# hammershock/3dgs-avatar-release

Hardware: AMD Instinct MI355X
Metric: render fps (fwd+bwd) @200k Gaussians 1024x1024 SH3 (higher is better)
Workload: dtype f32; 1 GPU; config3: 200k Gaussians, 1024x1024, SH deg 3, forward+backward; shs+scales+rotations inputs, L1 loss (L1 fused into the rasterizer: l1_target); tile_rect=1, l1=fused, long_lists=0, gaussians=200000, width=1024, height=1024, sh_degree=3, frames_per_rank=1857, total_frames=1857, ranks=1, backend=none, parallelism=frames sharded x1

## Files before the change

### 3dgs-avatar-release_amd/csrc/binning.hip

```cpp
#include "common.h"

__global__ __launch_bounds__(256) void first_pair_kernel(const uint32_t* __restrict__ tiles,
                                                         const uint32_t* __restrict__ wave_tiles, float* __restrict__ rec,
                                                         int P, unsigned long long* __restrict__ count,
                                                         unsigned long long* host_count) {
    __shared__ unsigned long long wb[4];
    const int tid = threadIdx.x, lane = tid & 63, wid = tid >> 6;
    const int w0 = 4 * (int)blockIdx.x;
    unsigned long long before = 0;
    for (int w = tid; w < w0; w += 256) before += wave_tiles[w];
#pragma unroll
    for (int d = 32; d >= 1; d >>= 1) before += __shfl_xor(before, d, 64);
    if (lane == 0) wb[wid] = before;
    const int i = blockIdx.x * 256 + tid;
    const uint32_t v = i < P ? tiles[i] : 0u;
    uint32_t x = v;
#pragma unroll
    for (int d = 1; d < 64; d <<= 1) {
        const uint32_t y = __shfl_up(x, d, 64);
        if (lane >= d) x += y;
    }
    __syncthreads();
    const unsigned long long block_base = (wb[0] + wb[1]) + (wb[2] + wb[3]);
    uint32_t woff = 0;
// ... 349 lines not shown
        uint32_t* __restrict__ nstash = &wmax[1];
        if (tid == 0) *nstash = 0u;
        __syncthreads();
        const uint32_t nx = (uint32_t)__popc(xmask);
        for (int pos = tid; pos < ntiles; pos += 1024) {
            const uint32_t ov = order[pos];
            if (!(ov >> 31)) continue;
            const int t = (int)(ov & 0x7FFFFFFFu);
            const uint32_t nch = (tile_work(ranges, keys, mode, t) + ch - 1u) / ch;
            const uint32_t u0 = atomicAdd(&wmax[0], nch);
            const uint32_t ph = (uint32_t)pos % (2u * nx);
            uint32_t pick = ph < nx ? ph : 2u * nx - 1u - ph, best = 0;
            for (uint32_t x = 0; x < 8; x++) {
                if ((xmask >> x) & 1u) {
                    if (pick == 0u) { best = x; break; }
                    pick--;
                }
            }
            const uint32_t i0 = atomicAdd(&wsum[8 + best], 4u * nch);
            const uint32_t k = atomicAdd(nstash, 1u);
            stash[4 * k] = (uint32_t)t;
            stash[4 * k + 1] = u0;
            stash[4 * k + 2] = i0 | (best << 28);
            stash[4 * k + 3] = nch;
        }
        __syncthreads();
        const uint32_t nk = *nstash;
        for (uint32_t k = (uint32_t)wid; k < nk; k += 16) {
            const uint32_t t = stash[4 * k], u0 = stash[4 * k + 1], ib = stash[4 * k + 2], nch = stash[4 * k + 3];
            uint32_t* __restrict__ items = ll.cw_items + (size_t)(ib >> 28) * (FWDC_MAX_UNITS * 4) + (ib & 0x0FFFFFFFu);
            for (uint32_t c = (uint32_t)lane; c < nch; c += 64) ll.cw_units[u0 + c] = make_uint2(t, c | (nch << 16));
            for (uint32_t i = (uint32_t)lane; i < 4u * nch; i += 64) items[i] = (u0 + (i >> 2)) * 4u + (i & 3u);
        }
    }
    if (ll.cw_hdr) {
        __syncthreads();
        if (tid == 0) {
            ll.cw_hdr[0] = (mode == 2 && ch) ? wmax[0] : 0u;
            ll.cw_hdr[1] = ch;
        }
        if (tid < 8) ll.cw_hdr[4 + tid] = (mode == 2 && ch) ? wsum[8 + tid] : 0u;
    }
}

template <bool HELD>
__global__ __launch_bounds__(1024) void tile_order_kernel(const uint2* __restrict__ ranges,
                                                          const uint32_t* __restrict__ keys, int mode, int ntiles,
                                                          uint32_t* __restrict__ order, const PairCount pc,
                                                          const FillJob fill, const LongLists ll) {
    if (blockIdx.x > 0) {
        if (fill.clean && *fill.clean == MARKS_CLEAN) return;
        const uint4 ones = make_uint4(0xFFFFFFFFu, 0xFFFFFFFFu, 0xFFFFFFFFu, 0xFFFFFFFFu);
        for (size_t k = (size_t)(blockIdx.x - 1) * 1024 + threadIdx.x; k < fill.quads; k += (size_t)(gridDim.x - 1) * 1024)
            if (fill.stream) store_stream(&fill.ptr[k], ones); else fill.ptr[k] = ones;
        return;
    }
    __shared__ uint32_t hist[1024];
    __shared__ uint32_t wmax[16];
    __shared__ uint32_t wsum[16];
    if (mode < 0) return;
    tile_order_body<HELD>(ranges, keys, mode, ntiles, order, pc, ll, hist, wmax, wsum);
}

#define BM_LD 33
#ifndef TW_STOP_AFTER
#define TW_STOP_AFTER 99
#endif
template <bool CW>
__global__ __launch_bounds__(TBK_THREADS) void tile_write_kernel(const uint4* __restrict__ ranklist,
                                                                 const uint32_t* __restrict__ seg_start, int P, int gx,
                                                                 int gy, int nbx, int nblocks, int nseg, int ntiles,
                                                                 const uint32_t* __restrict__ seg_cnt,
                                                                 const uint32_t* __restrict__ tile_tot,
                                                                 uint2* __restrict__ ranges, uint32_t* __restrict__ order,
                                                                 uint32_t* __restrict__ point_list, const PairCount pc,
                                                                 const LongLists ll) {
    __shared__ uint32_t m_id[TBK_BUF];
    __shared__ unsigned short m_rc[TBK_BUF];
    __shared__ uint32_t bitmap[TB_TILES * BM_LD];
    __shared__ uint32_t dst[TB_TILES];
    __shared__ uint32_t wcnt[TBK_WAVES];
    __shared__ unsigned long long sb_scratch[20];
    static_assert(TBK_THREADS == 1024 && TBK_WAVES == 16 && TB_H <= 4 && TB_TILES * BM_LD >= 1024 && TB_TILES >= 32, "the ordering job borrows bitmap / dst");
    if (blockIdx.x == 0) {
        if (CW) {
            if (ntiles <= 32 * 1024) tile_order_body<true>(nullptr, tile_tot, 2, ntiles, order, pc, ll, bitmap, dst, dst + 16);
            else tile_order_body<false>(nullptr, tile_tot, 2, ntiles, order, pc, ll, bitmap, dst, dst + 16);
        } else if (ntiles <= 32 * 1024) {
            tile_order_plain<true>(nullptr, tile_tot, 2, ntiles, order, pc, ll, bitmap, dst, dst + 16);
        } else {
            tile_order_plain<false>(nullptr, tile_tot, 2, ntiles, order, pc, ll, bitmap, dst, dst + 16);
        }
        return;
    }
    const int tid = threadIdx.x, lane = tid & 63, wid = tid >> 6;
    const int b = ((int)blockIdx.x - 1) % nblocks, sg = ((int)blockIdx.x - 1) / nblocks;
    const int r0 = min(P, (int)seg_start[sg] * 256), r1 = min(P, (int)seg_start[sg + 1] * 256);
    const int bx0 = (b % nbx) * TB_W, by0 = (b / nbx) * TB_H;
    const int bx1 = min(gx, bx0 + TB_W), by1 = min(gy, by0 + TB_H);
    const unsigned long long frame_pairs = *pc.dev;
    const bool fits = frame_pairs <= (unsigned long long)pc.cap;
    uint32_t my_dst = 0;
    {
        const int t_blk0 = by0 * gx + bx0;
        uint32_t part = 0;
        for (int t0 = 0; t0 < t_blk0; t0 += 4 * TBK_THREADS) {
            uint32_t v[4];
#pragma unroll
            for (int k = 0; k < 4; k++) v[k] = t0 + k * TBK_THREADS + tid < t_blk0 ? tile_tot[t0 + k * TBK_THREADS + tid] : 0u;
            part += (v[0] + v[1]) + (v[2] + v[3]);
        }
        const int ty = by0 + wid, tx = bx0 + lane;
        const bool row_ok = tid < TB_TILES && ty < by1;
        const int t_row0 = ty * gx + bx0, t = t_row0 + lane;
        const bool tile_ok = row_ok && tx < bx1;
        uint32_t tot = 0, pre = 0, rowsum = 0;
        if (row_ok) {
            for (int k = lane; k < gx; k += 64) rowsum += t_row0 + k < ntiles ? tile_tot[t_row0 + k] : 0u;
            if (tile_ok) {
                tot = tile_tot[t];
                for (int s0 = 0; s0 < sg; s0 += 8) {
                    uint32_t v[8];
#pragma unroll
                    for (int k = 0; k < 8; k++) v[k] = (s0 + k < sg) ? seg_cnt[(size_t)(s0 + k) * ntiles + t] : 0u;
#pragma unroll
                    for (int k = 0; k < 8; k++) pre += v[k];
                }
            }
        }
        part = wave_sum(part);
        rowsum = wave_sum(rowsum);
        uint32_t* s_part = reinterpret_cast<uint32_t*>(sb_scratch);
        if (lane == 0) {
            s_part[wid] = part;
            if (wid < TB_H) s_part[16 + wid] = rowsum;
        }
        __syncthreads();
        if (row_ok) {
            uint32_t before = 0;
            for (int w = 0; w < TBK_WAVES; w++) before += s_part[w];
            for (int r = 0; r < wid; r++) before += s_part[16 + r];
            const uint32_t x = wave_scan_incl(tot);
            const uint32_t first = before + x - tot;
            if (sg == 0 && tile_ok) ranges[t] = fits ? make_uint2(first, first + tot) : make_uint2(0u, 0u);
            my_dst = first + pre;
        }
        __syncthreads();
    }
    if (TW_STOP_AFTER <= 1) return;
    if (!fits || !point_list) return;
    for (int k = tid; k < TB_TILES * BM_LD; k += TBK_THREADS) bitmap[k] = 0u;
    uint4 e[TBK_LPL];
    auto load_trip = [&](const int rb) {
#pragma unroll
        for (int k = 0; k < TBK_LPL; k++) {
            const int r = rb + wid * (64 * TBK_LPL) + k * 64 + lane;
            e[k] = r < r1 ? ranklist[r] : make_uint4(0, 0, 0, 0);
        }
    };
    if (TW_STOP_AFTER <= 2) return;
    load_trip(r0);
    if (tid < TB_TILES) dst[tid] = my_dst;
    const unsigned long long lt_mask = (lane == 0) ? 0ull : (~0ull >> (64 - lane));
    int count = 0;
    const int grp = lane >> 4, gl = lane & 15;

    auto process_batch = [&](const int n) {
        const int nw = (n + 31) >> 5;
        for (int m0 = wid * 4; m0 < n; m0 += TBK_WAVES * 4) {
            const int m = m0 + grp;
            if (m < n) {
                const uint32_t rc = m_rc[m];
                const uint32_t lw = ((rc >> 8) & 63u) + 1u, lh = ((rc >> 14) & 3u) + 1u;
                const uint32_t area = lw * lh, lx = rc & 63u, ly = (rc >> 6) & 3u;
                for (uint32_t j = (uint32_t)gl; j < area; j += 16u) {
                    const uint32_t dy = (j >= lw ? 1u : 0u) + (j >= 2u * lw ? 1u : 0u) + (j >= 3u * lw ? 1u : 0u);
                    const uint32_t lt = (ly + dy) * TB_W + lx + (j - dy * lw);
                    atomicOr(&bitmap[lt * BM_LD + (m >> 5)], 1u << (m & 31));
                }
// ... 145 lines not shown
```

### 3dgs-avatar-release_amd/csrc/capi.hip

```cpp
#include "common.h"
#include "boundary.h"
#include <string.h>
#include <stdlib.h>
#include <atomic>
#include <chrono>
#include <mutex>
#include <vector>

static thread_local int g_last_hip = 0;
static thread_local const char* g_last_stage = "";
void gs_set_error(int hip_err, const char* stage) {
    g_last_hip = hip_err;
    g_last_stage = stage;
}

struct TuneSwitch {
    const char* name;
    int key, def;
    const char* env;
    bool (*ok)(int);
};
static const TuneSwitch k_tune[GS_TUNE_COUNT] = {
    {"xcd_map", GS_TUNE_XCD_MAP, 1, nullptr, nullptr},
    {"depth_sort", GS_TUNE_DEPTH_SORT, 1, nullptr, nullptr},
    {"nt_stores", GS_TUNE_NT_STORES, 1, nullptr, nullptr},
    {"bwd_chunks", GS_TUNE_BWD_CHUNKS, 1, nullptr, nullptr},
    {"fwd4", GS_TUNE_FWD4, 1, "GSPLAT_FWD4", nullptr},
    {"small_tiles", GS_TUNE_SMALL_TILES, BWD_CHUNK_MAX_TILES, nullptr, nullptr},
    {"shared_qlist", GS_TUNE_SHARED_QLIST, 1, nullptr, nullptr},
    {"ones_fast", GS_TUNE_ONES_FAST, 1, nullptr, nullptr},
    {"bwd_order", GS_TUNE_BWD_ORDER, 1, nullptr, nullptr},
    {"fwd_marks", GS_TUNE_FWD_MARKS, 1, nullptr, nullptr},
    {"fwdc_ch", GS_TUNE_FWDC_CH, (int)FWDC_CH_MIN, "GSPLAT_FWDC_CH", [](int v) { return v >= 64 && (v & (v - 1)) == 0; }},
    {"fwdc_div", GS_TUNE_FWDC_DIV, (int)FWD4_TOTAL_DIV, "GSPLAT_FWDC_DIV", [](int v) { return v >= 1; }},
};
struct TuneState {
    std::atomic<int> v[GS_TUNE_COUNT];
    TuneState() {
        for (const TuneSwitch& t : k_tune) {
            int value = t.def;
            if (const char* e = t.env ? getenv(t.env) : nullptr) {
                const int x = atoi(e);
                if (!t.ok || t.ok(x)) value = x;
            }
            v[t.key].store(value);
        }
    }
};
static TuneState& tune_state() {
    static TuneState st;
    return st;
}
int gs_tune_get(int key) {
    return (key >= 0 && key < GS_TUNE_COUNT) ? tune_state().v[key].load(std::memory_order_relaxed) : 0;
}

struct ProfRec { const char* name; hipEvent_t a, b; };
struct ProfState {
    bool on = false;
    bool armed = false;
    int nested = 0;
    char filter[32] = {0};
    std::vector<ProfRec> recs;
    std::vector<hipEvent_t> pool;
    hipEvent_t get() {
        if (!pool.empty()) { hipEvent_t e = pool.back(); pool.pop_back(); return e; }
        hipEvent_t e = nullptr;
        (void)hipEventCreate(&e);
        return e;
    }
};
static ProfState g_prof;
static std::mutex g_prof_mu;
bool profiling_on() { return g_prof.on; }
void gs_prof_begin(const char* stage, hipStream_t s) {
    if (!g_prof.on) return;
    std::lock_guard<std::mutex> lk(g_prof_mu);
    if (g_prof.armed) { g_prof.nested++; return; }
    g_prof.armed = g_prof.on && (g_prof.filter[0] == 0 || strcmp(g_prof.filter, stage) == 0);
    if (!g_prof.armed) return;
    ProfRec r{stage, g_prof.get(), g_prof.get()};
    (void)hipEventRecord(r.a, s);
    g_prof.recs.push_back(r);
}
void gs_prof_end(hipStream_t s) {
    if (!g_prof.on) return;
    std::lock_guard<std::mutex> lk(g_prof_mu);
    if (!g_prof.armed || g_prof.recs.empty()) return;
    if (g_prof.nested > 0) { g_prof.nested--; return; }
    (void)hipEventRecord(g_prof.recs.back().b, s);
    g_prof.armed = false;
}

static int validate(const GsFwdArgs* a) {
    if (!a) return GS_E_BAD_ARG;
    if (a->P < 0 || a->W <= 0 || a->H <= 0) return GS_E_BAD_ARG;
    if (!a->bg || !a->viewmatrix || !a->projmatrix || !a->campos) return GS_E_BAD_ARG;
    if (a->P > 0 && (!a->means3D || !a->opacities)) return GS_E_BAD_ARG;
    if ((a->shs != nullptr) == (a->colors_precomp != nullptr)) return GS_E_EXCLUSIVE;
    const bool sr = a->scales != nullptr && a->rotations != nullptr;
    if ((a->scales != nullptr) != (a->rotations != nullptr)) return GS_E_EXCLUSIVE;
    if (sr == (a->cov3D_precomp != nullptr)) return GS_E_EXCLUSIVE;
    if (a->shs) {
        if (a->sh_degree < 0 || a->sh_degree > 3) return GS_E_BAD_ARG;
        if (a->M < (a->sh_degree + 1) * (a->sh_degree + 1)) return GS_E_BAD_ARG;
        if (a->M > 16) return GS_E_BAD_ARG;
    }
    if (!aligned(a->rotations, 16)) return GS_E_BAD_ARG;
    if ((a->W + TILE - 1) / TILE > 0xFFFF || (a->H + TILE - 1) / TILE > 0xFFFF) return GS_E_TOO_LARGE;
    return GS_OK;
}

bool stream_is_capturing(void* stream) {
    hipStreamCaptureStatus st = hipStreamCaptureStatusNone;
    const hipError_t e = hipStreamIsCapturing((hipStream_t)stream, &st);
    if (e != hipSuccess) {
        (void)hipGetLastError();
        return e == hipErrorStreamCaptureImplicit || e == hipErrorStreamCaptureUnsupported || e == hipErrorStreamCaptureInvalidated;
    }
    return st != hipStreamCaptureStatusNone;
}

__global__ void zero_words_kernel(uint32_t* __restrict__ p, size_t words) {
    for (size_t k = (size_t)blockIdx.x * blockDim.x + threadIdx.x; k < words; k += (size_t)gridDim.x * blockDim.x) p[k] = 0u;
}
int gs_zero_async(void* ptr, size_t bytes, const char* stage, hipStream_t s) {
    const size_t words = bytes / 4;
    if (words == 0) return GS_OK;
    const size_t blocks = (words + 255) / 256;
    hipLaunchKernelGGL(zero_words_kernel, dim3((unsigned)(blocks < 1024 ? blocks : 1024)), dim3(256), 0, s, (uint32_t*)ptr, words);
    const hipError_t e = hipGetLastError();
    if (e != hipSuccess) { gs_set_error((int)e, stage); return GS_E_HIP; }
    return GS_OK;
}

__global__ __launch_bounds__(256) void clock_probe_kernel(unsigned long long* __restrict__ out, int iters, float seed, float* __restrict__ sink) {
    const unsigned long long t0 = __builtin_readcyclecounter(), r0 = __builtin_amdgcn_s_memrealtime();
    float a[8];
#pragma unroll
    for (int i = 0; i < 8; i++) a[i] = seed + (float)i + (float)threadIdx.x * 1e-3f;
    for (int it = 0; it < iters; it++) {
#pragma unroll
        for (int u = 0; u < 4; u++)
#pragma unroll
            for (int i = 0; i < 8; i++) a[i] = __builtin_fmaf(a[i], 1.0001f, 0.5f);
    }
    float sum = 0.f;
#pragma unroll
    for (int i = 0; i < 8; i++) sum += a[i];
    if (sum == 12345.678f) sink[0] = sum;
    if (threadIdx.x == 0) {
        const unsigned long long t1 = __builtin_readcyclecounter(), r1 = __builtin_amdgcn_s_memrealtime();
        atomicAdd(&out[0], t1 - t0);
        atomicAdd(&out[1], r1 - r0);
    }
}

__global__ __launch_bounds__(64) void xcc_probe_kernel(uint32_t* __restrict__ out) {
    if (threadIdx.x == 0) out[blockIdx.x] = xcc_id();
}

template <class Void, class VoidBin, class G, class B, class I, class Own>
static int frame_states(const GsFwdArgs* a, Void* geom, size_t geom_bytes, VoidBin* binning, size_t binning_bytes, Void* img,
                        size_t img_bytes, int64_t D, G* g, B* b, I* im, Own own) {
    int rc = validate(a);
    if (rc != GS_OK) return rc;
    if (!geom || !img || D < 0 || (D > 0 && !binning)) return GS_E_BAD_ARG;
    if ((rc = own()) != GS_OK) return rc;
    *g = geom_state(geom, a->P);
    *im = img_state(img, a->W, a->H, a->long_lists);
    *b = bin_state(D > 0 ? binning : nullptr, D);
    if (geom_bytes < g->total || img_bytes < im->total || (D > 0 && binning_bytes < b->total)) return GS_E_WORKSPACE;
    return GS_OK;
}

template <class T> static T* writable(T* p) { return p; }
template <class T> static T* writable(const T* p) { return const_cast<T*>(p); }
template <bool RO>
static QuadLists quad_lists(const ImgViewT<RO>& im, const BinView& b, int long_lists) {
    QuadLists ql;
    ql.qlist = b.qlist;
    ql.ncon_c = writable(im.ncon_c);
    ql.qcount = writable(im.qcount);
    ql.chunks = gs_tune_get(GS_TUNE_BWD_CHUNKS) ? im.bwd_chunks : 1;
    ql.four_waves = forward_small_image(im.ntiles, long_lists) ? 1 : 0;
    ql.ckpt = ql.chunks > 1 ? writable(im.ckpt) : nullptr;
    ql.ck_start = ql.chunks > 1 ? writable(im.ck_start) : nullptr;
    return ql;
}
template <bool RO>
static void quad_lists_chunked(QuadLists& ql, const ImgView& own, const ImgViewT<RO>& list) {
    ql.chunked = 1;
    ql.cw_hdr = list.cw_hdr;
    ql.cw_units = list.cw_units;
    ql.cw_items = list.cw_items;
    ql.cw_q = own.cw_q;
    ql.cw_flag = own.cw_flag;
    ql.cw_done = own.cw_done;
    ql.cw_rec = own.cw_rec;
}
static int sync_if_debug(const GsFwdArgs* a, const char* stage, hipStream_t s) {
    if (!a->debug) return GS_OK;
    const hipError_t e = hipStreamSynchronize(s);
// ... 390 lines not shown
        default: return GS_E_BAD_ARG;
    }
    return GS_OK;
}
int gs_image_field(void* img, int32_t W, int32_t H, int32_t field, void** out) {
    if (!img || !out) return GS_E_BAD_ARG;
    const ImgView im = img_state(img, W, H, 0);
    void* p = nullptr;
    switch (field) {
        case GS_IMG_RANGES: p = im.ranges; break;
        case GS_IMG_N_CONTRIB: p = im.n_contrib; break;
        case GS_IMG_FINAL_T: p = im.final_T; break;
        case GS_IMG_QCOUNT: p = im.qcount; break;
        case GS_IMG_NCON_C: p = im.ncon_c; break;
        case GS_IMG_ORDER: p = im.order; break;
        case GS_IMG_CW_HDR: p = im.cw_hdr; break;
        case GS_IMG_CW_UNITS: p = im.cw_units; break;
        case GS_IMG_CW_FLAG: p = im.cw_flag; break;
        case GS_IMG_CW_REC: p = im.cw_rec; break;
    }
    if (!p) return GS_E_BAD_ARG;
    *out = p;
    return GS_OK;
}

int gs_profile_enable(int on) {
    std::lock_guard<std::mutex> lk(g_prof_mu);
    g_prof.on = on != 0;
    return GS_OK;
}
int gs_profile_reserve(int n_events) {
    std::lock_guard<std::mutex> lk(g_prof_mu);
    hipEvent_t last = nullptr;
    while ((int)g_prof.pool.size() < n_events) {
        hipEvent_t e = nullptr;
        if (hipEventCreate(&e) != hipSuccess) return GS_E_HIP;
        (void)hipEventRecord(e, nullptr);
        last = e;
        g_prof.pool.push_back(e);
    }
    if (last) (void)hipEventSynchronize(last);
    return GS_OK;
}
int gs_profile_filter(const char* stage) {
    std::lock_guard<std::mutex> lk(g_prof_mu);
    memset(g_prof.filter, 0, sizeof(g_prof.filter));
    if (stage) strncpy(g_prof.filter, stage, sizeof(g_prof.filter) - 1);
    return GS_OK;
}
int gs_profile_collect(int max, const char** names, float* ms, int32_t* launches, int32_t* n_out) {
    if (max < 0 || !n_out || (max > 0 && (!names || !ms || !launches))) return GS_E_BAD_ARG;
    std::lock_guard<std::mutex> lk(g_prof_mu);
    int n = 0;
    for (auto& r : g_prof.recs) {
        float t = 0.f;
        hipError_t e = hipEventSynchronize(r.b);
        if (e == hipSuccess) e = hipEventElapsedTime(&t, r.a, r.b);
        if (e != hipSuccess) { gs_set_error((int)e, "profile.collect"); t = 0.f; }
        int k = 0;
        for (; k < n; k++) if (names[k] == r.name) break;
        if (k == n) {
            if (n < max) { names[n] = r.name; ms[n] = 0.f; launches[n] = 0; n++; } else k = -1;
        }
        if (k >= 0) { ms[k] += t; launches[k] += 1; }
        g_prof.pool.push_back(r.a);
        g_prof.pool.push_back(r.b);
    }
    g_prof.recs.clear();
    *n_out = n;
    return GS_OK;
}

int gs_tuning(const char* name, int value) {
    if (!name) return GS_E_BAD_ARG;
    for (const TuneSwitch& t : k_tune) {
        if (strcmp(name, t.name) != 0) continue;
        if (t.ok && !t.ok(value)) return GS_E_BAD_ARG;
        tune_state().v[t.key].store(value);
        return GS_OK;
    }
    return GS_E_BAD_ARG;
}

const char* gs_status_string(int code) {
    switch (code) {
        case GS_OK: return "ok";
        case GS_E_BAD_ARG: return "bad argument (null required pointer, non-positive size, unsupported SH degree / more than 16 SH coefficients, or rotations not 16-byte aligned)";
        case GS_E_EXCLUSIVE: return "provide exactly one of shs/colors_precomp and exactly one of (scales, rotations)/cov3D_precomp";
        case GS_E_TOO_LARGE: return "num_rendered or tile grid exceeds the supported index space";
        case GS_E_HIP: return "HIP error";
        case GS_E_WORKSPACE: return "state/workspace buffer smaller than gs_*_bytes requires";
        case GS_E_CAPTURE: return "the stream is being captured into a graph and this call is not capture-safe with these arguments (include/gsplat_mi355.h, \"Stream capture\"); nothing was enqueued";
        default: return "unknown status";
    }
}
int gs_last_hip_error(void) { return g_last_hip; }
const char* gs_last_stage(void) { return g_last_stage; }
const char* gs_build_info(void) { return "gsplat_mi355 gfx950 wave64 tile16 rec48"; }

}
```

### 3dgs-avatar-release_amd/csrc/common.h

```cpp
#pragma once
#include <hip/hip_runtime.h>
#include <stdint.h>
#include <stddef.h>
#include <type_traits>
#include "../../include/gsplat_mi355.h"

#define TILE 16
#define WAVE 64
#define REC_F 12
#define GS_MAX_PAIRS 0x3FFFFFFFll

static inline size_t align_up(size_t x, size_t a) { return (x + a - 1) / a * a; }

#define SORT_ITEMS 4096
#define SORT_SMALL_N (1 << 20)
#define SORT_TOTALS_REPL 16
static inline size_t sort_table_words(size_t n) {
    const size_t items = n <= (size_t)SORT_SMALL_N ? 1024 : SORT_ITEMS;
    return (size_t)256 * ((n + items - 1) / items + 4 * SORT_TOTALS_REPL);
}
#define SCAN_ITEMS 2048

#ifndef DS_ITEMS
#define DS_ITEMS 2048
// ... 9 lines not shown
#define TB_MAX_SEG 64
enum { COUNT_PAIRS = 0, COUNT_NOT_ONES = 2, COUNT_ZERO_BYTES = 24 };
struct GeomLayout {
    size_t rec, depths, tiles, clamped, key0, key1, val0, val1, ranklist, chunk_pairs, wsum, wkmin, wkmax, hist, count,
        ds_tmp, ds_tmp2, ds_cnt, ds_pre, ds_tot, ds_loc, ds_grp, ds_range, seg_start, total;
    int nblk_sort, nwaves, ds_nb, ds_blocks;
};
static inline GeomLayout geom_layout(int P) {
    GeomLayout L;
    size_t o = 0;
    size_t n = (size_t)(P > 0 ? P : 1);
    auto take = [&](size_t bytes) { size_t at = o; o = align_up(o + bytes, 256); return at; };
    L.nblk_sort = (int)((n + SORT_ITEMS - 1) / SORT_ITEMS);
    L.nwaves = (int)((n + 255) / 256) * 4;
    L.rec = take(n * REC_F * 4);
    L.depths = take(n * 4);
    L.tiles = take(n * 4);
    L.clamped = take(n * 4);
    L.key0 = take(n * 4);
    L.key1 = take(n * 4);
    L.val0 = take(n * 4);
    L.val1 = take(n * 4);
    L.ranklist = take(n * 16);
    L.chunk_pairs = take(((n + 255) / 256) * 4);
    L.wsum = take((size_t)L.nwaves * 4);
    L.wkmin = take((size_t)L.nwaves * 4);
    L.wkmax = take((size_t)L.nwaves * 4);
    L.hist = take(sort_table_words(n) * 4);
    L.count = take(64);
    L.ds_nb = ds_buckets(P);
    L.ds_blocks = (int)((n + DS_ITEMS - 1) / DS_ITEMS);
    L.ds_tmp = take(n * 8);
    L.ds_tmp2 = take(n * 8);
    L.ds_cnt = take((size_t)L.ds_blocks * (L.ds_nb + 1) * 4);
    L.ds_pre = take((size_t)L.ds_blocks * (L.ds_nb + 1) * 4);
    L.ds_tot = take((size_t)(L.ds_nb + 1) * 4);
    L.ds_loc = take((size_t)(L.ds_nb + 1) * 4);
    L.ds_grp = take((size_t)((L.ds_nb + 1 + 63) / 64) * 4);
    L.ds_range = take(16);
    L.seg_start = take((size_t)(TB_MAX_SEG + 2) * 4);
    L.total = o;
    return L;
}

struct BinLayout {
    size_t point_list, qlist, marks, marks_flag, total;
};
static inline BinLayout bin_layout(int64_t D) {
    BinLayout L;
    size_t o = 0;
    size_t n = (size_t)(D > 0 ? D : 1);
    auto take = [&](size_t bytes) { size_t at = o; o = align_up(o + bytes, 256); return at; };
    L.point_list = take(n * 4);
    L.qlist = take(n * 16);
    L.marks = take(n * 16);
    L.marks_flag = take(4);
    L.total = o;
    return L;
}

#define TB_W 64
#ifndef TB_H
#define TB_H 4
#endif
#define TB_TILES (TB_W * TB_H)
struct BinGrid { int nbx, nby, nblocks, nseg_max; };
static inline BinGrid bin_grid(int gx, int gy) {
    BinGrid G;
    G.nbx = (gx + TB_W - 1) / TB_W;
    G.nby = (gy + TB_H - 1) / TB_H;
    G.nblocks = G.nbx * G.nby;
#ifndef TB_TARGET_WGS
#define TB_TARGET_WGS 512
#endif
    int s = (TB_TARGET_WGS + G.nblocks - 1) / G.nblocks;
    G.nseg_max = s < 1 ? 1 : (s > TB_MAX_SEG ? TB_MAX_SEG : s);
    return G;
}
static inline int bin_segments(const BinGrid& G, int P) {
    int s = (P + 1023) / 1024;
    if (s < 1) s = 1;
    return s < G.nseg_max ? s : G.nseg_max;
}

enum { GS_TUNE_XCD_MAP = 0, GS_TUNE_DEPTH_SORT = 1, GS_TUNE_NT_STORES = 2, GS_TUNE_BWD_CHUNKS = 3, GS_TUNE_FWD4 = 4, GS_TUNE_SMALL_TILES = 5, GS_TUNE_SHARED_QLIST = 6, GS_TUNE_ONES_FAST = 7, GS_TUNE_BWD_ORDER = 8, GS_TUNE_FWD_MARKS = 9, GS_TUNE_FWDC_CH = 10, GS_TUNE_FWDC_DIV = 11, GS_TUNE_COUNT = 12 };
int gs_tune_get(int key);

#define BWD_CH 128
#define BWD_KMAX 16
#define BWD_CHUNK_MAX_TILES 2048
#define FWD4_MAX_TILES 2048
#define FWD4_MIN_LIST 512u
#ifndef FWD4_TOTAL_DIV
#define FWD4_TOTAL_DIV 320ull
#endif

#define FWDC_CH_MIN 256u
#define FWDC_SPARSE_PAIRS 524288ull
#define FWDC_MAX_UNITS 4096
#define FWDC_MAX_TILES (FWDC_MAX_UNITS / 2)
#define FWDC_Q_WORDS (8 * FWDC_MAX_UNITS * 4)
#define FWDC_Q_BYTES ((size_t)FWDC_Q_WORDS * 4 + 64)
#ifdef FWDC_PROF
#define FWDC_SLOTS 9
#else
#define FWDC_SLOTS 8
#endif
#define FWDC_DEAD 0x80000000u
#define FWDC_SPIN_MAX (1 << 16)
struct ImgLayout {
    size_t ranges, n_contrib, final_T, ncon_c, tile_nmax, order, seg_cnt, tile_tot, all_ones, cw_flag, cw_done, cw_q, tile_zero_bytes, l1_part, ckpt, ck_start, cw_hdr, cw_units, cw_items, cw_rec, total;
    int gx, gy, bwd_chunks;
};
static inline bool few_long_lists_mode(int ntiles, int long_lists) {
    return ntiles <= gs_tune_get(GS_TUNE_SMALL_TILES) || long_lists != 0;
}
static inline ImgLayout img_layout(int W, int H, int long_lists = 0) {
    ImgLayout L;
    size_t o = 0;
    auto take = [&](size_t bytes) { size_t at = o; o = align_up(o + bytes, 256); return at; };
    L.gx = (W + TILE - 1) / TILE;
    L.gy = (H + TILE - 1) / TILE;
    const size_t nt = (size_t)L.gx * L.gy;
    L.ranges = take(nt * 8);
    L.n_contrib = take((size_t)W * H * 4);
    L.final_T = take((size_t)W * H * 4);
    L.ncon_c = take((size_t)W * H * 4);
    L.tile_nmax = take(nt * 16);
    L.order = take(nt * 4);
    L.seg_cnt = take(nt * 4 * (size_t)bin_grid(L.gx, L.gy).nseg_max);
    L.tile_tot = take(nt * 4);
    L.all_ones = take(4);
    L.tile_zero_bytes = L.all_ones + 4 - L.tile_tot;
    const bool fl = few_long_lists_mode((int)nt, long_lists);
    const bool cw = fl && gs_tune_get(GS_TUNE_FWD4) == 2;
    L.cw_flag = L.cw_done = L.cw_q = 0;
    if (cw) {
        L.cw_flag = take((size_t)FWDC_MAX_UNITS * 4 * 4);
        L.cw_done = take(nt * 16);
        L.cw_q = take(FWDC_Q_BYTES);
        L.tile_zero_bytes = L.cw_q + FWDC_Q_BYTES - L.tile_tot;
    }
    L.l1_part = take(nt * 16);
    L.bwd_chunks = fl ? BWD_KMAX : 1;
    L.ckpt = take(nt * 4 * (size_t)(L.bwd_chunks - 1) * 64 * 16);
    L.ck_start = take(nt * 4 * (size_t)L.bwd_chunks * 4);
    L.cw_hdr = L.cw_units = L.cw_items = L.cw_rec = 0;
    if (cw) {
        L.cw_hdr = take(64);
        L.cw_units = take((size_t)FWDC_MAX_UNITS * 8);
        L.cw_items = take((size_t)FWDC_Q_WORDS * 4);
        L.cw_rec = take((size_t)FWDC_MAX_UNITS * 4 * FWDC_SLOTS * 64 * 4);
    }
    L.total = o;
    return L;
}

template <bool RO>
struct StateCarve {
    typename std::conditional<RO, const char, char>::type* base;
    StateCarve(typename std::conditional<RO, const void, void>::type* state) : base(static_cast<decltype(base)>(state)) {}
    template <class T>
    void operator()(T*& field, size_t offset, bool present = true) const {
        field = (base && present) ? reinterpret_cast<T*>(base + offset) : nullptr;
    }
};
template <bool RO>
struct GeomViewT {
    template <class T> using ptr = typename std::conditional<RO, const T, T>::type*;
// ... 403 lines not shown
```

### 3dgs-avatar-release_amd/csrc/gaussian_bwd.hip

```cpp
#include "common.h"
#include "gs_math.h"
#include "blend.h"

#ifndef GB_THREADS
#define GB_THREADS 256
#endif

__global__ __launch_bounds__(256) void segment_reduce_kernel(int P, const int32_t* __restrict__ radii,
                                                             const float4* __restrict__ rec,
                                                             const uint32_t* __restrict__ tiles,
                                                             const uint32_t* __restrict__ q8,
                                                             const float4* __restrict__ qrows,
                                                             float4* __restrict__ sums, uint32_t* __restrict__ marks_flag) {
    const int t = blockIdx.x * blockDim.x + threadIdx.x;
    if (t == 0 && marks_flag) *marks_flag = 0u;
    const int i = t >> 4, j = t & 15;
    const int rs = j >> 1, h = j & 1;
    float a0 = 0.f, a1 = 0.f, a2 = 0.f, a3 = 0.f, a8 = 0.f;
    const bool in = i < P;
    float4 r0 = make_float4(0.f, 0.f, 0.f, 0.f), r1 = r0;
    if (in && radii[i] > 0) {
        const uint32_t off = __float_as_uint(rec[(size_t)i * 3 + 2].y);
        const uint32_t nrows = 4u * tiles[i];
        if (j < 2) {
// ... 221 lines not shown
                            dx += SH_C3[0] * SHC(9) * 3.f * 2.f * xy + SH_C3[1] * SHC(10) * yz + SH_C3[2] * SHC(11) * -2.f * xy +
                                  SH_C3[3] * SHC(12) * -3.f * 2.f * xz + SH_C3[4] * SHC(13) * (-3.f * xx + 4.f * zz - yy) +
                                  SH_C3[5] * SHC(14) * 2.f * xz + SH_C3[6] * SHC(15) * 3.f * (xx - yy);
                            dy += SH_C3[0] * SHC(9) * 3.f * (xx - yy) + SH_C3[1] * SHC(10) * xz + SH_C3[2] * SHC(11) * (-3.f * yy + 4.f * zz - xx) +
                                  SH_C3[3] * SHC(12) * -3.f * 2.f * yz + SH_C3[4] * SHC(13) * -2.f * xy +
                                  SH_C3[5] * SHC(14) * -2.f * yz + SH_C3[6] * SHC(15) * -3.f * 2.f * xy;
                            dz += SH_C3[1] * SHC(10) * xy + SH_C3[2] * SHC(11) * 4.f * 2.f * yz + SH_C3[3] * SHC(12) * 3.f * (2.f * zz - xx - yy) +
                                  SH_C3[4] * SHC(13) * 4.f * 2.f * xz + SH_C3[5] * SHC(14) * (xx - yy);
                        }
                    }
                }
                for (int k = (deg + 1) * (deg + 1); k < M; k++) GSH(k) = 0.f;
#undef SHC
#undef GSH
                ddir[0] += dx * g;
                ddir[1] += dy * g;
                ddir[2] += dz * g;
            }
            const float sum2 = dox * dox + doy * doy + doz * doz;
            const float invsum32 = 1.0f / sqrtf(sum2 * sum2 * sum2);
            gm[0] += ((+sum2 - dox * dox) * ddir[0] - doy * dox * ddir[1] - doz * dox * ddir[2]) * invsum32;
            gm[1] += (-dox * doy * ddir[0] + (sum2 - doy * doy) * ddir[1] - doz * doy * ddir[2]) * invsum32;
            gm[2] += (-dox * doz * ddir[0] - doy * doz * ddir[1] + (sum2 - doz * doz) * ddir[2]) * invsum32;
        }
        if (!cov3D_precomp) {
            float R[3][3];
            quat_to_R(q, R);
            const float sv[3] = {scale_modifier * sc.x, scale_modifier * sc.y, scale_modifier * sc.z};
            const float dS[3][3] = {{gc[0], 0.5f * gc[1], 0.5f * gc[2]},
                                    {0.5f * gc[1], gc[3], 0.5f * gc[4]},
                                    {0.5f * gc[2], 0.5f * gc[4], gc[5]}};
            float L[3][3], dL[3][3], dR[3][3];
#pragma unroll
            for (int r_ = 0; r_ < 3; r_++)
#pragma unroll
                for (int c_ = 0; c_ < 3; c_++) L[r_][c_] = R[r_][c_] * sv[c_];
#pragma unroll
            for (int r_ = 0; r_ < 3; r_++)
#pragma unroll
                for (int c_ = 0; c_ < 3; c_++)
                    dL[r_][c_] = 2.0f * (dS[r_][0] * L[0][c_] + dS[r_][1] * L[1][c_] + dS[r_][2] * L[2][c_]);
#pragma unroll
            for (int c_ = 0; c_ < 3; c_++) {
                gs[c_] = R[0][c_] * dL[0][c_] + R[1][c_] * dL[1][c_] + R[2][c_] * dL[2][c_];
#pragma unroll
                for (int r_ = 0; r_ < 3; r_++) dR[r_][c_] = dL[r_][c_] * sv[c_];
            }
            const float r = q.x, x = q.y, y = q.z, z = q.w;
            gq[0] = 2 * z * (dR[1][0] - dR[0][1]) + 2 * y * (dR[0][2] - dR[2][0]) + 2 * x * (dR[2][1] - dR[1][2]);
            gq[1] = 2 * y * (dR[0][1] + dR[1][0]) + 2 * z * (dR[0][2] + dR[2][0]) + 2 * r * (dR[2][1] - dR[1][2]) - 4 * x * (dR[2][2] + dR[1][1]);
            gq[2] = 2 * x * (dR[0][1] + dR[1][0]) + 2 * r * (dR[0][2] - dR[2][0]) + 2 * z * (dR[2][1] + dR[1][2]) - 4 * y * (dR[2][2] + dR[0][0]);
            gq[3] = 2 * r * (dR[1][0] - dR[0][1]) + 2 * x * (dR[0][2] + dR[2][0]) + 2 * y * (dR[2][1] + dR[1][2]) - 4 * z * (dR[1][1] + dR[0][0]);
        }
    } else if (shs) {
        float* gsh = sh_tile + threadIdx.x * ld;
        for (int k = 0; k < M * 3; k++) gsh[k] = 0.f;
    }
    dL_dmeans3D[3 * i] = gm[0];
    dL_dmeans3D[3 * i + 1] = gm[1];
    dL_dmeans3D[3 * i + 2] = gm[2];
#pragma unroll
    for (int k = 0; k < 6; k++) dL_dcov3D[6 * i + k] = gc[k];
    if (dL_dscales) {
        dL_dscales[3 * i] = gs[0];
        dL_dscales[3 * i + 1] = gs[1];
        dL_dscales[3 * i + 2] = gs[2];
    }
    if (dL_drotations) reinterpret_cast<float4*>(dL_drotations)[i] = make_float4(gq[0], gq[1], gq[2], gq[3]);
    }
    if (shs) {
        __syncthreads();
        sh_tile_store(dL_dsh + (size_t)row0 * M * 3, sh_tile, nrows, M * 3, ld);
    }
}

int launch_gaussian_backward(const GsFwdArgs& a, const int32_t* radii, const float* rec, const uint32_t* tiles,
                             const uint32_t* clamped, const uint32_t* q8, const float* qrows, float* sums,
                             uint32_t* marks_flag, const GsGrads& g, hipStream_t s) {
    const float fy = a.H / (2.0f * a.tanfovy), fx = a.W / (2.0f * a.tanfovx);
    hipLaunchKernelGGL(segment_reduce_kernel, dim3((unsigned)(((size_t)a.P * 16 + 255) / 256)), dim3(256), 0, s, a.P, radii,
                       reinterpret_cast<const float4*>(rec), tiles, q8,
                       reinterpret_cast<const float4*>(qrows), reinterpret_cast<float4*>(sums), marks_flag);
    GS_LAUNCH_CHECK("segment_reduce", a.debug, s);
    const size_t lds = a.shs ? (size_t)GB_THREADS * ((3 * a.M) | 1) * sizeof(float) : 0;
    hipLaunchKernelGGL(a.antialiasing ? gaussian_bwd_kernel<true> : gaussian_bwd_kernel<false>,
                       dim3((a.P + GB_THREADS - 1) / GB_THREADS), dim3(GB_THREADS), lds, s, a.P, a.sh_degree, a.M, a.means3D,
                       a.scales, a.scale_modifier, a.rotations, a.shs, a.cov3D_precomp, a.viewmatrix, a.projmatrix,
                       a.campos, a.W, a.H, a.tanfovx, a.tanfovy, fx, fy, radii, clamped,
                       reinterpret_cast<const float4*>(sums), g.dL_dmeans3D, g.dL_dmeans2D,
                       g.dL_dsh, g.dL_dcolors, g.dL_dopacity, g.dL_dscales, g.dL_drotations, g.dL_dcov3D,
                       reinterpret_cast<const float4*>(rec));
    GS_LAUNCH_CHECK("gaussian_backward", a.debug, s);
    return GS_OK;
}
```

### 3dgs-avatar-release_amd/csrc/gs_math.h

```cpp
#pragma once
#include <hip/hip_runtime.h>
#include <stdint.h>

#define SH_C0 0.28209479177387814f
#define SH_C1 0.4886025119029199f
__device__ __constant__ static const float SH_C2[5] = {1.0925484305920792f, -1.0925484305920792f, 0.31539156525252005f,
                                                       -1.0925484305920792f, 0.5462742152960396f};
__device__ __constant__ static const float SH_C3[7] = {-0.5900435899266435f, 2.890611442640554f,
                                                       -0.4570457994644658f, 0.3731763325901154f,
                                                       -0.4570457994644658f, 1.445305721320277f,
                                                       -0.5900435899266435f};

__device__ __forceinline__ float3 xform4x3(const float3 p, const float* m) {
    return make_float3(m[0] * p.x + m[4] * p.y + m[8] * p.z + m[12], m[1] * p.x + m[5] * p.y + m[9] * p.z + m[13],
                       m[2] * p.x + m[6] * p.y + m[10] * p.z + m[14]);
}
__device__ __forceinline__ float4 xform4x4(const float3 p, const float* m) {
    return make_float4(m[0] * p.x + m[4] * p.y + m[8] * p.z + m[12], m[1] * p.x + m[5] * p.y + m[9] * p.z + m[13],
                       m[2] * p.x + m[6] * p.y + m[10] * p.z + m[14], m[3] * p.x + m[7] * p.y + m[11] * p.z + m[15]);
}

__device__ __forceinline__ void quat_to_R(const float4 q, float R[3][3]) {
    const float r = q.x, x = q.y, y = q.z, z = q.w;
    R[0][0] = 1.f - 2.f * (y * y + z * z);
// ... 94 lines not shown
    const float thr = 2.0f * ln_upper_bound(x) + 0.002f;
    const float cond = (cov_a * cov_c) / det;
    const float widen = 1.0f + cond * 1.9073486e-6f;
    if (!(det > 0.0f) || !(widen <= 2.0f)) {
        *hx = *hy = 1.0e7f;
        return true;
    }
    const float thr_w = thr * widen;
    *hx = fminf(sqrtf(thr_w * cov_a), 1.0e7f);
    *hy = fminf(sqrtf(thr_w * cov_c), 1.0e7f);
    return true;
}

__device__ __forceinline__ float3 sh_eval_dir(int deg, const float x, const float y, const float z,
                                              const float* __restrict__ sh, uint32_t* clamped) {
    float out[3];
    uint32_t cl = 0;
#pragma unroll
    for (int c = 0; c < 3; c++) {
#define SHC(k) sh[(k) * 3 + c]
        float r = SH_C0 * SHC(0);
        if (deg > 0) {
            r = r - SH_C1 * y * SHC(1) + SH_C1 * z * SHC(2) - SH_C1 * x * SHC(3);
            if (deg > 1) {
                const float xx = x * x, yy = y * y, zz = z * z, xy = x * y, yz = y * z, xz = x * z;
                r = r + SH_C2[0] * xy * SHC(4) + SH_C2[1] * yz * SHC(5) + SH_C2[2] * (2.0f * zz - xx - yy) * SHC(6) +
                    SH_C2[3] * xz * SHC(7) + SH_C2[4] * (xx - yy) * SHC(8);
                if (deg > 2) {
                    r = r + SH_C3[0] * y * (3.0f * xx - yy) * SHC(9) + SH_C3[1] * xy * z * SHC(10) +
                        SH_C3[2] * y * (4.0f * zz - xx - yy) * SHC(11) +
                        SH_C3[3] * z * (2.0f * zz - 3.0f * xx - 3.0f * yy) * SHC(12) +
                        SH_C3[4] * x * (4.0f * zz - xx - yy) * SHC(13) + SH_C3[5] * z * (xx - yy) * SHC(14) +
                        SH_C3[6] * x * (xx - 3.0f * yy) * SHC(15);
                }
            }
        }
#undef SHC
        r += 0.5f;
        if (r < 0.f) cl |= (1u << c);
        out[c] = fmaxf(r, 0.f);
    }
    *clamped = cl;
    return make_float3(out[0], out[1], out[2]);
}

__device__ __forceinline__ float3 sh_to_rgb(int deg, const float3 mean, const float3 campos, const float* __restrict__ sh,
                                            uint32_t* clamped) {
    const float dx = mean.x - campos.x, dy = mean.y - campos.y, dz = mean.z - campos.z;
    const float len = sqrtf(dx * dx + dy * dy + dz * dz);
    return sh_eval_dir(deg, dx / len, dy / len, dz / len, sh, clamped);
}

struct Mat3 { float m[9]; };

__device__ __forceinline__ void view_dir(const float* __restrict__ xyz, const float* __restrict__ campos,
                                         const float* __restrict__ R_fwd, int ms, int rs, int use_noise, const Mat3& noise, int i,
                                         float d[3], float* len) {
    float v[3] = {xyz[3 * (size_t)i] - campos[0], xyz[3 * (size_t)i + 1] - campos[1], xyz[3 * (size_t)i + 2] - campos[2]};
    if (R_fwd) {
        const float* R = R_fwd + ms * (size_t)i;
        const float w[3] = {R[0] * v[0] + R[rs] * v[1] + R[2 * rs] * v[2], R[1] * v[0] + R[rs + 1] * v[1] + R[2 * rs + 1] * v[2],
                            R[2] * v[0] + R[rs + 2] * v[1] + R[2 * rs + 2] * v[2]};
        v[0] = w[0]; v[1] = w[1]; v[2] = w[2];
    }
    if (use_noise) {
        const float w[3] = {v[0] * noise.m[0] + v[1] * noise.m[3] + v[2] * noise.m[6],
                            v[0] * noise.m[1] + v[1] * noise.m[4] + v[2] * noise.m[7],
                            v[0] * noise.m[2] + v[1] * noise.m[5] + v[2] * noise.m[8]};
        v[0] = w[0]; v[1] = w[1]; v[2] = w[2];
    }
    const float l = sqrtf(v[0] * v[0] + v[1] * v[1] + v[2] * v[2]);
    d[0] = v[0]; d[1] = v[1]; d[2] = v[2];
    *len = l;
}

__device__ __forceinline__ int sh_tile_ld(int M) { return (3 * M) | 1; }
__device__ __forceinline__ void sh_tile_load(const float* __restrict__ g, float* __restrict__ lds, int nrows, int rf,
                                             int ld) {
    if ((rf & 3) == 0 && ((uintptr_t)g & 15u) == 0) {
        const int rf4 = rf >> 2, total4 = nrows * rf4;
        int r = (int)threadIdx.x / rf4, c = (int)threadIdx.x - r * rf4;
        const int dr = (int)blockDim.x / rf4, dc = (int)blockDim.x - dr * rf4;
        const float4* g4 = reinterpret_cast<const float4*>(g);
        for (int e0 = threadIdx.x; e0 < total4; e0 += 4 * (int)blockDim.x) {
            float4 v[4];
#pragma unroll
            for (int u = 0; u < 4; u++) v[u] = e0 + u * (int)blockDim.x < total4 ? g4[e0 + u * (int)blockDim.x] : make_float4(0.f, 0.f, 0.f, 0.f);
#pragma unroll
            for (int u = 0; u < 4; u++) {
                if (e0 + u * (int)blockDim.x < total4) {
                    float* d = lds + r * ld + 4 * c;
                    d[0] = v[u].x; d[1] = v[u].y; d[2] = v[u].z; d[3] = v[u].w;
                }
                r += dr;
                c += dc;
                if (c >= rf4) { c -= rf4; r++; }
            }
        }
        return;
    }
    const int total = nrows * rf;
    int r = (int)threadIdx.x / rf, c = (int)threadIdx.x - r * rf;
    const int dr = (int)blockDim.x / rf, dc = (int)blockDim.x - dr * rf;
    for (int e = threadIdx.x; e < total; e += blockDim.x) {
        lds[r * ld + c] = g[e];
        r += dr;
        c += dc;
        if (c >= rf) { c -= rf; r++; }
    }
}
__device__ __forceinline__ void sh_tile_store(float* __restrict__ g, const float* __restrict__ lds, int nrows, int rf,
                                              int ld) {
    if ((rf & 3) == 0 && ((uintptr_t)g & 15u) == 0) {
        const int rf4 = rf >> 2, total4 = nrows * rf4;
        int r = (int)threadIdx.x / rf4, c = (int)threadIdx.x - r * rf4;
        const int dr = (int)blockDim.x / rf4, dc = (int)blockDim.x - dr * rf4;
        float4* g4 = reinterpret_cast<float4*>(g);
        for (int e = threadIdx.x; e < total4; e += blockDim.x) {
            const float* d = lds + r * ld + 4 * c;
            g4[e] = make_float4(d[0], d[1], d[2], d[3]);
            r += dr;
            c += dc;
            if (c >= rf4) { c -= rf4; r++; }
        }
        return;
    }
    const int total = nrows * rf;
    int r = (int)threadIdx.x / rf, c = (int)threadIdx.x - r * rf;
    const int dr = (int)blockDim.x / rf, dc = (int)blockDim.x - dr * rf;
    for (int e = threadIdx.x; e < total; e += blockDim.x) {
        g[e] = lds[r * ld + c];
        r += dr;
        c += dc;
        if (c >= rf) { c -= rf; r++; }
    }
}
```

### include/gsplat_mi355.h

```cpp
#ifndef GSPLAT_MI355_H
#define GSPLAT_MI355_H

#include <stddef.h>
#include <stdint.h>

#ifdef __cplusplus
extern "C" {
#endif

#define GS_OK 0
#define GS_E_BAD_ARG (-1)
#define GS_E_EXCLUSIVE (-2)
#define GS_E_TOO_LARGE (-3)
#define GS_E_HIP (-4)
#define GS_E_WORKSPACE (-5)
#define GS_E_CAPTURE (-6)


typedef struct GsFwdArgs {
    int32_t P;
    int32_t sh_degree;
    int32_t M;
    int32_t W, H;
    const float* bg;
// ... 333 lines not shown
    const float* b[GS_MLP_MAX_LAYERS];
    float* dW[GS_MLP_MAX_LAYERS];
    float* db[GS_MLP_MAX_LAYERS];
    float *dx, *dcond;
} GsMlpArgs;
int gs_mlp_workspace_bytes(const GsMlpArgs* a, int32_t backward, size_t* out);
int gs_mlp_forward(const GsMlpArgs* a, float* y, float* acts, void* workspace, size_t workspace_bytes, void* stream);
int gs_mlp_backward(const GsMlpArgs* a, const float* acts, const float* dL_dy, void* workspace, size_t workspace_bytes,
                    void* stream);

#define GS_LPIPS_LAYERS 13
#define GS_LPIPS_TAPS 5
#define GS_LPIPS_MIN_SIZE 16
#define GS_LPIPS_MAX_SIZE 2048
#define GS_LPIPS_WS_FORWARD 0
#define GS_LPIPS_WS_SAVED 1
#define GS_LPIPS_WS_BACKWARD 2
typedef struct GsLpipsArgs {
    int32_t H, W, normalize, need_grad0, need_grad1;
    int64_t cs0, rs0, cs1, rs1;
    const float *in0, *in1, *packed;
    const float* weight[GS_LPIPS_LAYERS];
    const float* bias[GS_LPIPS_LAYERS];
    const float* lin[GS_LPIPS_TAPS];
    const float *shift, *scale;
} GsLpipsArgs;
int gs_lpips_packed_bytes(size_t* out);
int gs_lpips_pack_weights(const GsLpipsArgs* a, void* packed, size_t packed_bytes, void* stream);
int gs_lpips_workspace_bytes(int32_t H, int32_t W, int32_t need_grad0, int32_t need_grad1, int32_t which, size_t* out);
int gs_lpips_forward(const GsLpipsArgs* a, float* loss, float* per_tap, void* saved, size_t saved_bytes, void* workspace,
                     size_t workspace_bytes, void* stream);
int gs_lpips_backward(const GsLpipsArgs* a, const float* dL_dloss, float* d_in0, float* d_in1, const void* saved,
                      size_t saved_bytes, void* workspace, size_t workspace_bytes, void* stream);
int gs_lpips_conv(const float* packed, int32_t layer, int32_t backward, int32_t normalize, int32_t H, int32_t W, const float* in,
                  int64_t in_cs, int64_t in_rs, const float* mask, float* out, void* stream);
int gs_lpips_pool(int32_t backward, int32_t H, int32_t W, int32_t C, const float* in, const float* g, const float* dp, float* out,
                  void* stream);

enum GsGeomField {
    GS_GEOM_DEPTHS = 0,
    GS_GEOM_TILES = 1,
    GS_GEOM_REC = 2,
    GS_GEOM_CLAMPED = 3,
    GS_GEOM_SORTED_IDX = 4,
    GS_GEOM_COUNT = 5,
    GS_GEOM_FIELDS = 6
};
enum GsBinningField {
    GS_BIN_POINT_LIST = 0,
    GS_BIN_QLIST = 1,
    GS_BIN_FIELDS = 2
};
enum GsImageField {
    GS_IMG_RANGES = 0,
    GS_IMG_N_CONTRIB = 1,
    GS_IMG_FINAL_T = 2,
    GS_IMG_QCOUNT = 3,
    GS_IMG_NCON_C = 4,
    GS_IMG_ORDER = 5,
    GS_IMG_CW_HDR = 6,
    GS_IMG_CW_UNITS = 7,
    GS_IMG_CW_FLAG = 8,
    GS_IMG_CW_REC = 9,
    GS_IMG_FIELDS = 10
};
int gs_geom_field(void* geom, int32_t P, int32_t field, void** out);
int gs_binning_field(void* binning, int64_t num_rendered, int32_t W, int32_t H, int32_t field, void** out);
int gs_image_field(void* img, int32_t W, int32_t H, int32_t field, void** out);
int gs_image_bytes_for(const GsFwdArgs* a, size_t* out);

int gs_profile_reserve(int n_events);
int gs_profile_enable(int on);
int gs_profile_filter(const char* stage);
int gs_profile_collect(int max, const char** names, float* ms, int32_t* launches, int32_t* n_out);

int gs_pair_stats(const GsFwdArgs* a, const void* geom, size_t geom_bytes, const void* binning, size_t binning_bytes,
                  const void* img, size_t img_bytes, int64_t num_rendered, uint64_t* counts, void* stream);

int gs_clock_probe(uint64_t* ticks, int32_t iters, void* stream);

int gs_xcc_probe(uint32_t* xcc, int32_t n_blocks, void* stream);

int gs_tuning(const char* name, int value);
const char* gs_status_string(int code);
int gs_last_hip_error(void);
const char* gs_last_stage(void);
const char* gs_build_info(void);

#ifdef __cplusplus
}
#endif
#endif
```

Before: 1809 frames/s.

## Pick gaussian backward block size from residency, widen SH tile load unroll

Chooses between 64 and 256 threads for the gaussian backward kernel by estimating how many resident workgroup generations each size needs, using occupancy queries that are cached per kernel. Widens the SH tile load unroll from 4 to 12 float4 loads in flight per thread. Moves the tile-ordering job from block 0 to the last block of the tile write kernel. The aims are fewer tail waves in the backward pass and more memory-level parallelism, at the cost of higher register pressure and host-side occupancy queries on first use.

```diff
diff --git a/3dgs-avatar-release_amd/csrc/binning.hip b/3dgs-avatar-release_amd/csrc/binning.hip
--- a/3dgs-avatar-release_amd/csrc/binning.hip
+++ b/3dgs-avatar-release_amd/csrc/binning.hip
@@ -455,7 +455,7 @@
     __shared__ uint32_t wcnt[TBK_WAVES];
     __shared__ unsigned long long sb_scratch[20];
     static_assert(TBK_THREADS == 1024 && TBK_WAVES == 16 && TB_H <= 4 && TB_TILES * BM_LD >= 1024 && TB_TILES >= 32, "the ordering job borrows bitmap / dst");
-    if (blockIdx.x == 0) {
+    if (blockIdx.x == gridDim.x - 1) {
         if (CW) {
             if (ntiles <= 32 * 1024) tile_order_body<true>(nullptr, tile_tot, 2, ntiles, order, pc, ll, bitmap, dst, dst + 16);
             else tile_order_body<false>(nullptr, tile_tot, 2, ntiles, order, pc, ll, bitmap, dst, dst + 16);
@@ -467,7 +467,7 @@
         return;
     }
     const int tid = threadIdx.x, lane = tid & 63, wid = tid >> 6;
-    const int b = ((int)blockIdx.x - 1) % nblocks, sg = ((int)blockIdx.x - 1) / nblocks;
+    const int b = (int)blockIdx.x % nblocks, sg = (int)blockIdx.x / nblocks;
     const int r0 = min(P, (int)seg_start[sg] * 256), r1 = min(P, (int)seg_start[sg + 1] * 256);
     const int bx0 = (b % nbx) * TB_W, by0 = (b / nbx) * TB_H;
     const int bx1 = min(gx, bx0 + TB_W), by1 = min(gy, by0 + TB_H);
diff --git a/3dgs-avatar-release_amd/csrc/capi.hip b/3dgs-avatar-release_amd/csrc/capi.hip
--- a/3dgs-avatar-release_amd/csrc/capi.hip
+++ b/3dgs-avatar-release_amd/csrc/capi.hip
@@ -33,6 +33,8 @@
     {"fwd_marks", GS_TUNE_FWD_MARKS, 1, nullptr, nullptr},
     {"fwdc_ch", GS_TUNE_FWDC_CH, (int)FWDC_CH_MIN, "GSPLAT_FWDC_CH", [](int v) { return v >= 64 && (v & (v - 1)) == 0; }},
     {"fwdc_div", GS_TUNE_FWDC_DIV, (int)FWD4_TOTAL_DIV, "GSPLAT_FWDC_DIV", [](int v) { return v >= 1; }},
+    {"resident_wgs", GS_TUNE_RESIDENT_WGS, 0, nullptr, [](int v) { return v >= 0; }},
+    {"gb_threads", GS_TUNE_GB_THREADS, 0, nullptr, [](int v) { return v == 0 || v == 64 || v == 256; }},
 };
 struct TuneState {
     std::atomic<int> v[GS_TUNE_COUNT];
@@ -119,6 +121,38 @@
         return e == hipErrorStreamCaptureImplicit || e == hipErrorStreamCaptureUnsupported || e == hipErrorStreamCaptureInvalidated;
     }
     return st != hipStreamCaptureStatusNone;
+}
+
+struct ResidentRec { int dev; const void* kernel; int threads; size_t lds; int wgs; };
+static std::vector<ResidentRec> g_resident;
+static std::mutex g_resident_mu;
+int gs_resident_wgs(const void* kernel, int threads, size_t dyn_lds, int fallback, hipStream_t s) {
+    const int forced = gs_tune_get(GS_TUNE_RESIDENT_WGS);
+    if (forced > 0) return forced;
+    int dev = -1;
+    if (hipGetDevice(&dev) != hipSuccess) { (void)hipGetLastError(); return fallback; }
+    {
+        std::lock_guard<std::mutex> lk(g_resident_mu);
+        for (const ResidentRec& r : g_resident)
+            if (r.dev == dev && r.kernel == kernel && r.threads == threads && r.lds == dyn_lds) return r.wgs;
+    }
+    if (stream_is_capturing(s)) return fallback;
+    int cus = 0, per_cu = 0;
+    hipFuncAttributes fa;
+    if (hipDeviceGetAttribute(&cus, hipDeviceAttributeMultiprocessorCount, dev) != hipSuccess ||
+        hipFuncGetAttributes(&fa, kernel) != hipSuccess ||
+        hipOccupancyMaxActiveBlocksPerMultiprocessor(&per_cu, kernel, threads, dyn_lds) != hipSuccess || cus <= 0 || per_cu <= 0) {
+        (void)hipGetLastError();
+        return fallback;
+    }
+    const size_t lds = fa.sharedSizeBytes + dyn_lds;
+    const int waves = (threads + 63) / 64;
+    if (lds > 0 && (size_t)per_cu > 163840 / lds) per_cu = (int)(163840 / lds);
+    if (per_cu > 32 / waves) per_cu = 32 / waves;
+    const int wgs = per_cu > 0 ? cus * per_cu : fallback;
+    std::lock_guard<std::mutex> lk(g_resident_mu);
+    g_resident.push_back(ResidentRec{dev, kernel, threads, dyn_lds, wgs});
+    return wgs;
 }
 
 __global__ void zero_words_kernel(uint32_t* __restrict__ p, size_t words) {
@@ -675,6 +709,10 @@
     return GS_E_BAD_ARG;
 }
 
+int32_t gs_gaussian_bwd_threads(int32_t n, int32_t resident64, int32_t resident256) {
+    return gaussian_bwd_threads(n, resident64, resident256);
+}
+
 const char* gs_status_string(int code) {
     switch (code) {
         case GS_OK: return "ok";
diff --git a/3dgs-avatar-release_amd/csrc/common.h b/3dgs-avatar-release_amd/csrc/common.h
--- a/3dgs-avatar-release_amd/csrc/common.h
+++ b/3dgs-avatar-release_amd/csrc/common.h
@@ -115,9 +115,20 @@
     if (s < 1) s = 1;
     return s < G.nseg_max ? s : G.nseg_max;
 }
-
-enum { GS_TUNE_XCD_MAP = 0, GS_TUNE_DEPTH_SORT = 1, GS_TUNE_NT_STORES = 2, GS_TUNE_BWD_CHUNKS = 3, GS_TUNE_FWD4 = 4, GS_TUNE_SMALL_TILES = 5, GS_TUNE_SHARED_QLIST = 6, GS_TUNE_ONES_FAST = 7, GS_TUNE_BWD_ORDER = 8, GS_TUNE_FWD_MARKS = 9, GS_TUNE_FWDC_CH = 10, GS_TUNE_FWDC_DIV = 11, GS_TUNE_COUNT = 12 };
+#define GB_RESIDENT_FALLBACK 768
+#define GB_RESIDENT64_FALLBACK 3328
+
+enum { GS_TUNE_XCD_MAP = 0, GS_TUNE_DEPTH_SORT = 1, GS_TUNE_NT_STORES = 2, GS_TUNE_BWD_CHUNKS = 3, GS_TUNE_FWD4 = 4, GS_TUNE_SMALL_TILES = 5, GS_TUNE_SHARED_QLIST = 6, GS_TUNE_ONES_FAST = 7, GS_TUNE_BWD_ORDER = 8, GS_TUNE_FWD_MARKS = 9, GS_TUNE_FWDC_CH = 10, GS_TUNE_FWDC_DIV = 11, GS_TUNE_RESIDENT_WGS = 12, GS_TUNE_GB_THREADS = 13, GS_TUNE_COUNT = 14 };
 int gs_tune_get(int key);
+
+int gs_resident_wgs(const void* kernel, int threads, size_t dyn_lds, int fallback, hipStream_t s);
+static inline int gaussian_bwd_threads(int N, int resident64, int resident256) {
+    auto generations = [](long long n, int per, int resident) {
+        const long long wgs = (n + per - 1) / per, r = resident > 0 ? resident : 1;
+        return (wgs + r - 1) / r;
+    };
+    return generations(N, 64, resident64) < generations(N, 256, resident256) ? 64 : 256;
+}
 
 #define BWD_CH 128
 #define BWD_KMAX 16
diff --git a/3dgs-avatar-release_amd/csrc/gaussian_bwd.hip b/3dgs-avatar-release_amd/csrc/gaussian_bwd.hip
--- a/3dgs-avatar-release_amd/csrc/gaussian_bwd.hip
+++ b/3dgs-avatar-release_amd/csrc/gaussian_bwd.hip
@@ -327,9 +327,16 @@
                        reinterpret_cast<const float4*>(rec), tiles, q8,
                        reinterpret_cast<const float4*>(qrows), reinterpret_cast<float4*>(sums), marks_flag);
     GS_LAUNCH_CHECK("segment_reduce", a.debug, s);
-    const size_t lds = a.shs ? (size_t)GB_THREADS * ((3 * a.M) | 1) * sizeof(float) : 0;
-    hipLaunchKernelGGL(a.antialiasing ? gaussian_bwd_kernel<true> : gaussian_bwd_kernel<false>,
-                       dim3((a.P + GB_THREADS - 1) / GB_THREADS), dim3(GB_THREADS), lds, s, a.P, a.sh_degree, a.M, a.means3D,
+    const auto kernel = a.antialiasing ? gaussian_bwd_kernel<true> : gaussian_bwd_kernel<false>;
+    const size_t row_bytes = a.shs ? (size_t)((3 * a.M) | 1) * sizeof(float) : 0;
+    int threads = gs_tune_get(GS_TUNE_GB_THREADS);
+    if (threads == 0) {
+        const void* k = reinterpret_cast<const void*>(kernel);
+        threads = gaussian_bwd_threads(a.P, gs_resident_wgs(k, 64, 64 * row_bytes, GB_RESIDENT64_FALLBACK, s),
+                                       gs_resident_wgs(k, GB_THREADS, GB_THREADS * row_bytes, GB_RESIDENT_FALLBACK, s));
+    }
+    const size_t lds = (size_t)threads * row_bytes;
+    hipLaunchKernelGGL(kernel, dim3((a.P + threads - 1) / threads), dim3(threads), lds, s, a.P, a.sh_degree, a.M, a.means3D,
                        a.scales, a.scale_modifier, a.rotations, a.shs, a.cov3D_precomp, a.viewmatrix, a.projmatrix,
                        a.campos, a.W, a.H, a.tanfovx, a.tanfovy, fx, fy, radii, clamped,
                        reinterpret_cast<const float4*>(sums), g.dL_dmeans3D, g.dL_dmeans2D,
diff --git a/3dgs-avatar-release_amd/csrc/gs_math.h b/3dgs-avatar-release_amd/csrc/gs_math.h
--- a/3dgs-avatar-release_amd/csrc/gs_math.h
+++ b/3dgs-avatar-release_amd/csrc/gs_math.h
@@ -200,12 +200,13 @@
         int r = (int)threadIdx.x / rf4, c = (int)threadIdx.x - r * rf4;
         const int dr = (int)blockDim.x / rf4, dc = (int)blockDim.x - dr * rf4;
         const float4* g4 = reinterpret_cast<const float4*>(g);
-        for (int e0 = threadIdx.x; e0 < total4; e0 += 4 * (int)blockDim.x) {
-            float4 v[4];
-#pragma unroll
-            for (int u = 0; u < 4; u++) v[u] = e0 + u * (int)blockDim.x < total4 ? g4[e0 + u * (int)blockDim.x] : make_float4(0.f, 0.f, 0.f, 0.f);
-#pragma unroll
-            for (int u = 0; u < 4; u++) {
+        constexpr int U = 12;
+        for (int e0 = threadIdx.x; e0 < total4; e0 += U * (int)blockDim.x) {
+            float4 v[U];
+#pragma unroll
+            for (int u = 0; u < U; u++) v[u] = e0 + u * (int)blockDim.x < total4 ? g4[e0 + u * (int)blockDim.x] : make_float4(0.f, 0.f, 0.f, 0.f);
+#pragma unroll
+            for (int u = 0; u < U; u++) {
                 if (e0 + u * (int)blockDim.x < total4) {
                     float* d = lds + r * ld + 4 * c;
                     d[0] = v[u].x; d[1] = v[u].y; d[2] = v[u].z; d[3] = v[u].w;
diff --git a/include/gsplat_mi355.h b/include/gsplat_mi355.h
--- a/include/gsplat_mi355.h
+++ b/include/gsplat_mi355.h
@@ -439,6 +439,7 @@
 int gs_xcc_probe(uint32_t* xcc, int32_t n_blocks, void* stream);
 
 int gs_tuning(const char* name, int value);
+int32_t gs_gaussian_bwd_threads(int32_t n, int32_t resident64, int32_t resident256);
 const char* gs_status_string(int code);
 int gs_last_hip_error(void);
 const char* gs_last_stage(void);
```

After: 1814 frames/s, median of 6. Within noise of the previous version (+0.3%).
